# nelpy/ghost

Hardware: NVIDIA B200
Metric: cwt_output_coeffs_per_sec (higher is better)
Workload: dtype f32

## Files before the change

ghost_b200/csrc/fast_path.cu:

```cuda
#include "plan.h"
#include "common.cuh"
#include "multiplier.cuh"
#include <algorithm>
#include <atomic>
#include <cmath>
#include <cstdio>
#include <cstdlib>
#include <map>
#include <type_traits>

namespace gcwt {

constexpr int kMaxFastLevel = 14;
constexpr int kMaxFullScales = 64;
constexpr double kMaxHaloFrac = 0.45;

__constant__ float c_halfband[kHalfbandOdd];
constexpr int kSmallCoef = (2 + 4 + 8) * kInterpT;
__constant__ float c_interp_small[kSmallCoef];
constexpr int kWideCoef = (4 + 8) * kWideT;
__constant__ float c_interp_wide[kWideCoef];

static double bessel_i0(double x) {
    double sum = 1.0, term = 1.0;
// ... 96 lines not shown

static int full_extent(const gcwt_plan* p, const PlanResponses& pr, int s) {
    const double* g = pr.full(s);
    const double e_tot = filter_energy(p, p->scales[s], kFullN);
    double e_in = 0.0;
    int m = 0;
    for (int nmu = 2; nmu <= 8; nmu *= 2) {
        for (; m < nmu * kBins; ++m) e_in += g[m] * g[m];
        if ((1.0 - e_in / e_tot) < p->band_tol * p->band_tol) return nmu;
    }
    return 16;
}

static int band_width_bins(const gcwt_plan* p, const PlanResponses& pr, int s, int level) {
    const double* g = pr.level(s, level);
    const double e_tot = filter_energy(p, p->scales[s], (int64_t)kChunkDec << level);
    const double budget = 0.5 * p->band_tol * p->band_tol * e_tot;
    int lo = 0, hi = kBins - 1;
    double acc = 0.0;
    while (lo < hi && acc + g[lo] * g[lo] < budget) { acc += g[lo] * g[lo]; ++lo; }
    acc = 0.0;
    while (hi > lo && acc + g[hi] * g[hi] < budget) { acc += g[hi] * g[hi]; --hi; }
    return hi - lo + 1;
}

static int choose_level(const gcwt_plan* p, const PlanResponses& pr, int s) {
    const ScaleInfo& sc = p->scales[s];
    if (!(p->flags & GCWT_FLAG_FORCE_GENERIC)) {
        int lo = kMinFastLevel;
        while (lo <= kMaxFastLevel && (double)(sc.L - 1) > kMaxHaloFrac * (double)((int64_t)kChunkDec << lo)) ++lo;
        int hi = std::min(kMaxFastLevel, ilog2_ceil(sc.L) + 1);
        for (int lev = hi; lev >= lo; --lev)
            if (band_fits(p, pr, s, lev)) return lev;
        if ((double)(sc.L - 1) <= kMaxHaloFrac * kFullN) return -1;
    }
    return -2;
}

static void class_geometry(FastClass& fc) {
    const int64_t d = fc.level >= 0 ? (int64_t(1) << fc.level) : 1;
    const int64_t align = std::max<int64_t>(d, 16);
    const int taps = fc.wide ? kWideT : kInterpT;
    const int64_t lead = fc.interp ? (int64_t)(taps / 2 - 1) << fc.log2u : 0;
    const int64_t tail = fc.interp ? (int64_t)(taps / 2 + 1) << fc.log2u : 0;
    fc.offset = ((fc.lmax / 2 + lead + align - 1) / align) * align;
    fc.hop = ((fc.nc_full - (fc.lmax - 1) / 2 - tail - fc.offset) / align) * align;
// ... 208 lines not shown
    p->guard_gain_h = gain;
    p->guard_q_h = q;
    return GCWT_OK;
}

int fast_plan_build(gcwt_plan* p) {
    design_halfband(p->halfband_odd);
    { int rc = upload_constants(p); if (rc) return rc; }
    {
        std::vector<float2> tw(kFullN);
        for (int k = 0; k < kFullN; ++k) {
            const double a = -2.0 * M_PI * (double)k / (double)kFullN;
            tw[k] = make_float2((float)std::cos(a), (float)std::sin(a));
        }
        GCWT_CUDA_OK(cudaMalloc((void**)&p->d_twiddle, sizeof(float2) * kFullN));
        GCWT_CUDA_OK(cudaMemcpy(p->d_twiddle, tw.data(), sizeof(float2) * kFullN, cudaMemcpyHostToDevice));
    }
    PlanResponses pr;
    { int rc = compute_plan_responses(p, pr); if (rc) return rc; }
    std::vector<double> hb((size_t)(kMaxFastLevel + 1) * kBins, 1.0);
    for (int j = 1; j <= kMaxFastLevel; ++j)
        for (int m = 0; m < kBins; ++m)
            hb[(size_t)j * kBins + m] = halfband_gain(p->halfband_odd, 2.0 * M_PI * (double)m / (double)((int64_t)kChunkDec << j));
    std::map<int, std::vector<int>> by_level;
    p->max_level = 0;
    for (int s = 0; s < p->n_scales; ++s) {
        ScaleInfo& sc = p->scales[s];
        sc.level = choose_level(p, pr, s);
        if (sc.level == -2) p->generic_ids.push_back(s);
        else by_level[sc.level].push_back(s);
        p->max_level = std::max(p->max_level, sc.level);
    }
    for (auto& kv : by_level) {
        const int level = kv.first;
        const std::vector<int>& ids = kv.second;
        const int cap = level >= 0 ? kMaxClassScales : kMaxFullScales;
        for (size_t i0 = 0; i0 < ids.size(); i0 += cap) {
            p->classes.emplace_back();
            FastClass& fc = p->classes.back();
            fc.level = level;
            fc.nc_full = level >= 0 ? ((int64_t)kChunkDec << level) : kFullN;
            fc.scale_ids.assign(ids.begin() + i0, ids.begin() + std::min(ids.size(), i0 + cap));
            fc.lmax = 1;
            for (int id : fc.scale_ids) fc.lmax = std::max(fc.lmax, p->scales[id].L);
            const bool may_interp = p->out_kind != GCWT_OUT_COMPLEX && !(p->flags & GCWT_FLAG_NO_INTERP);
            fc.interp = level >= kInterpMinLevel && may_interp;
            fc.log2u = level - 1;
            int wmax = 1;
            if (level >= 0)
                for (int id : fc.scale_ids) wmax = std::max(wmax, band_width_bins(p, pr, id, level));
            if (may_interp && level >= 2 && level <= kWideMaxLevel) {
                if (512.0 / (double)wmax >= kWideMinOs) { fc.interp = true; fc.wide = true; fc.log2u = level; }
            }
            class_geometry(fc);
            if (fc.hop <= 0) { set_error("planner: non-positive hop"); return GCWT_ERR_ARG; }
            if (fc.wide) {
                const int64_t d = int64_t(1) << level, align = std::max<int64_t>(d, 16), nc2 = 2 * fc.nc_full;
                const int64_t lead = (int64_t)(kWideT / 2 - 1) << fc.log2u, tail = (int64_t)(kWideT / 2 + 1) << fc.log2u;
                fc.offset2 = ((fc.lmax / 2 + lead + align - 1) / align) * align;
                fc.hop2 = ((nc2 - (fc.lmax - 1) / 2 - tail - fc.offset2) / align) * align;
                const int ns2 = (int)fc.scale_ids.size();
                std::vector<float2> tab2((size_t)ns2 * 2 * kBins);
                for (int i = 0; i < ns2; ++i) {
                    const ScaleInfo& sc = p->scales[fc.scale_ids[i]];
                    const double* gsrc = pr.wide2(fc.scale_ids[i], level);
                    for (int m = 0; m < 2 * kBins; ++m) {
                        double g = gsrc[m] / (double)(2 * kChunkDec);
                        for (int j = 1; j <= level; ++j)
                            g /= halfband_gain(p->halfband_odd, 2.0 * M_PI * (double)m / (double)((int64_t)(2 * kChunkDec) << j));
                        double re = g, im = 0.0;
                        if ((sc.L & 1) == 0) {
                            const double ph = -M_PI * (double)m / (double)nc2;
                            re = g * std::cos(ph);
                            im = g * std::sin(ph);
                        }
                        tab2[(size_t)i * 2 * kBins + m] = make_float2((float)re, (float)im);
                    }
                }
                GCWT_CUDA_OK(cudaMalloc((void**)&fc.d_table2, sizeof(float2) * tab2.size()));
                GCWT_CUDA_OK(cudaMemcpy(fc.d_table2, tab2.data(), sizeof(float2) * tab2.size(), cudaMemcpyHostToDevice));
            }
            const int nb = level >= 0 ? kBins : kFullN;
            const int ns = (int)fc.scale_ids.size();
            std::vector<float2> tab((size_t)ns * nb);
            for (int i = 0; i < ns; ++i) {
                const ScaleInfo& sc = p->scales[fc.scale_ids[i]];
                const double* gsrc = level >= 0 ? pr.level(fc.scale_ids[i], level) : pr.full(fc.scale_ids[i]);
                for (int m = 0; m < nb; ++m) {
                    double g = gsrc[m];
                    if (level >= 0) {
                        for (int j = 1; j <= level; ++j) g /= hb[(size_t)j * kBins + m];
                        g /= (double)kChunkDec;
                    } else {
                        g /= (double)kFullN;
                    }
                    double re = g, im = 0.0;
                    if ((sc.L & 1) == 0) {
                        const double ph = -M_PI * (double)m / (double)fc.nc_full;
                        re = g * std::cos(ph);
                        im = g * std::sin(ph);
                    }
                    tab[(size_t)i * nb + m] = make_float2((float)re, (float)im);
                }
            }
            GCWT_CUDA_OK(cudaMalloc((void**)&fc.d_table, sizeof(float2) * tab.size()));
            GCWT_CUDA_OK(cudaMemcpy(fc.d_table, tab.data(), sizeof(float2) * tab.size(), cudaMemcpyHostToDevice));
            if (fc.interp) {
                std::vector<float> coef;
                if (fc.wide) {
                    design_interpolator(fc.log2u, coef, kWideT, kWideMinOs);
                } else {
                    const double os = std::min(8.0, std::max(kInterpMinOs, 0.98 * 1024.0 / (double)wmax));
                    design_interpolator(fc.log2u, coef, kInterpT, os);
                }
                GCWT_CUDA_OK(cudaMalloc((void**)&fc.d_coef, sizeof(float) * coef.size()));
                GCWT_CUDA_OK(cudaMemcpy(fc.d_coef, coef.data(), sizeof(float) * coef.size(), cudaMemcpyHostToDevice));
            }
            if (level < 0) {
                for (int id : fc.scale_ids) fc.scale_nmu.push_back(full_extent(p, pr, id));
                GCWT_CUDA_OK(cudaMalloc((void**)&fc.d_scale_nmu, sizeof(int32_t) * ns));
                GCWT_CUDA_OK(cudaMemcpy(fc.d_scale_nmu, fc.scale_nmu.data(), sizeof(int32_t) * ns, cudaMemcpyHostToDevice));
            }
            GCWT_CUDA_OK(cudaMalloc((void**)&fc.d_scale_ids, sizeof(int32_t) * ns));
            GCWT_CUDA_OK(cudaMemcpy(fc.d_scale_ids, fc.scale_ids.data(), sizeof(int32_t) * ns, cudaMemcpyHostToDevice));
        }
    }
    if (p->guard && !p->classes.empty()) {
        if (p->max_level + 2 >= kGuardLevels || (int)p->classes.size() > 64) p->guard = false;
        else { int rc = guard_plan_build(p, pr, hb); if (rc) return rc; }
    } else {
        p->guard = false;
    }
    return GCWT_OK;
}

void fast_plan_free(gcwt_plan* p) {
    if (p->d_guard_gain) cudaFree(p->d_guard_gain);
    if (p->d_guard_q) cudaFree(p->d_guard_q);
    if (p->d_guard_class) cudaFree(p->d_guard_class);
    if (p->d_guard_acc) cudaFree(p->d_guard_acc);
    if (p->d_guard_pow) cudaFree(p->d_guard_pow);
    if (p->d_guard_flags) cudaFree(p->d_guard_flags);
    if (p->h_guard_flags) cudaFreeHost(p->h_guard_flags);
    if (p->ev_guard) cudaEventDestroy(p->ev_guard);
    p->d_guard_gain = p->d_guard_q = nullptr; p->d_guard_class = nullptr; p->d_guard_acc = nullptr;
    p->d_guard_pow = nullptr; p->d_guard_flags = p->h_guard_flags = nullptr; p->ev_guard = nullptr;
    for (auto& fc : p->classes) {
        if (fc.d_table) cudaFree(fc.d_table);
        if (fc.d_table2) cudaFree(fc.d_table2);
        if (fc.d_scale_ids) cudaFree(fc.d_scale_ids);
        if (fc.d_coef) cudaFree(fc.d_coef);
        if (fc.d_scale_nmu) cudaFree(fc.d_scale_nmu);
    }
    p->classes.clear();
}

constexpr int kPyrTile = 1024;

template <typename TIn, bool FIRST>
__global__ void __launch_bounds__(256)
pyramid_kernel(const TIn* __restrict__ in, int64_t in_stride, int64_t in_lo, int64_t in_hi,
               const double* __restrict__ means, float* __restrict__ out, int64_t out_stride,
               int64_t out_lo, int64_t out_len,
               double* __restrict__ acc, int acc_stride, int level, int64_t seg_in, int64_t seg_out) {
    static_assert(kHalfbandT == 19, "tile indexing below assumes kMid == 9");
    constexpr int kMid = (kHalfbandT - 1) / 2;
    constexpr int kEv = kPyrTile + 2 * kMid + 2 + 4;
    constexpr int kOdShift = 12 - kMid;
    __shared__ __align__(16) float ev[kEv];
    __shared__ __align__(16) float ods[kEv + 16];
    const int c = blockIdx.y;
    const int64_t i0 = out_lo + (int64_t)blockIdx.x * kPyrTile;
    const int64_t u0 = 2 * i0 - kHalfbandT;
    const TIn* src = in + (int64_t)c * in_stride - (FIRST ? 0 : in_lo);
    typedef typename std::conditional<std::is_same<TIn, float>::value, float, double>::type TSub;
// ... 63 lines not shown
}

struct FusedParams {
    const void* src;
    int64_t src_stride;
    int64_t src_lo, src_hi;
    const double* means;
    int log2d;
    int p_cols;
    int log2p;
    float inv_nc;
    int64_t offset, hop, n_chunks, n;
    int n_scales;
    const int32_t* scale_ids;
    const float2* table;
    void* out;
    int64_t s_stride, c_stride;
    int iters;
    int units_per_chunk;
    int log2u;
    const float* coef;
    const float2* twf;
    const int32_t* scale_nmu;
    double* acc;
    int acc_stride;
    int class_idx;
    float ech_weight;
    float* pow;
    int pow_stride;
    float pow_weight;
    int guard_every;
    int q_mode;
};

__device__ __forceinline__ float2 tw_pos(const float2* __restrict__ twf, int k) {
    const float2 t = __ldg(twf + (k & (kFullN - 1)));
    return make_float2(t.x, -t.y);
}

__device__ __forceinline__ float sqrt_abs_approx(float v) {
    float r;
    asm("sqrt.approx.ftz.f32 %0, %1;" : "=f"(r) : "f"(fabsf(v)));
    return r;
}

__device__ __forceinline__ float sqrt_approx(float v) {
// ... 53 lines not shown
#pragma unroll
    for (int w = 0; w < 8; ++w) t += scratch[w];
    return t * (1.0f / (float)(NV * 256));
}

template <int NV>
__device__ __forceinline__ void chunk_energy_add(const float* v, float cm, float* scratch, double* dst, float weight) {
    float s = 0.f;
#pragma unroll
    for (int k = 0; k < NV; ++k) { const float d = v[k] - cm; s = fmaf(d, d, s); }
#pragma unroll
    for (int o = 16; o > 0; o >>= 1) s += __shfl_xor_sync(0xffffffffu, s, o);
    __syncthreads();
    if ((threadIdx.x & 31) == 0) scratch[threadIdx.x >> 5] = s;
    __syncthreads();
    if (threadIdx.x == 0) {
        float t = 0.f;
#pragma unroll
        for (int w = 0; w < 8; ++w) t += scratch[w];
        atomicAdd(dst, (double)(t * weight));
    }
}

template <bool PAIRED>
__device__ __forceinline__ void guard_pow_add(const float2* a, unsigned own, float* counter) {
    float pw = 0.f;
#pragma unroll
    for (int k = 0; k < 16; ++k) {
        const float v = a[k].x * a[k].x + a[k].y * a[k].y;
        pw += (own >> k & 1u) ? v : 0.f;
    }
    pw += __shfl_xor_sync(0xffffffffu, pw, 16);
    if (!PAIRED) pw += __shfl_xor_sync(0xffffffffu, pw, 8);
    pw += __shfl_xor_sync(0xffffffffu, pw, 4);
    pw += __shfl_xor_sync(0xffffffffu, pw, 2);
    pw += __shfl_xor_sync(0xffffffffu, pw, 1);
    const unsigned lane = threadIdx.x & 31u;
    if ((lane & (PAIRED ? 23u : 31u)) == 0) atomicAdd(counter, pw);
}

__device__ __forceinline__ float2* smem_fft1024_forward(float2* a, float2* b, const float2* __restrict__ tw) {
    constexpr int M = 256;
    const int j = threadIdx.x;
    float2 w[4][3];
#pragma unroll
    for (int p = 1; p < 5; ++p) {
        const int ns = 1 << (2 * p);
        const int idx = (j & (ns - 1)) * ((kFullN / 4) / ns);
#pragma unroll
        for (int r = 0; r < 3; ++r) w[p - 1][r] = __ldg(tw + (r + 1) * idx);
    }
#pragma unroll
    for (int p = 0; p < 5; ++p) {
        const int ns = 1 << (2 * p);
        const int k = j & (ns - 1);
        float2 v0 = a[j], v1 = a[j + M], v2 = a[j + 2 * M], v3 = a[j + 3 * M];
        if (p > 0) {
            v1 = cmul(v1, w[p - 1][0]);
            v2 = cmul(v2, w[p - 1][1]);
            v3 = cmul(v3, w[p - 1][2]);
        }
// ... 122 lines not shown
        const unsigned mask = valid_mask(rel, lp + 4, own_lo, own_hi);
        for (int s = 0; s < prm.n_scales; ++s) {
            float2 a[16];
            const float2* z = Zs + s * kBins + g;
#pragma unroll
            for (int i = 0; i < 16; ++i) a[i] = cmul(z[16 * i], R[i]);
            dft16<+1>(a);
            float2* e = ex + buf * 4096 + (g * 16) * 16 + r;
            e[0] = a[0];
#pragma unroll
            for (int k = 1; k < 16; ++k) e[k * 16] = cmul(a[k], tw[k]);
            __syncthreads();
            if (pend >= 0 && tid == 0) {
                atomicAdd(pow_c + s_ids[pend], s_pow[pend & 1] * (float)iters * prm.pow_weight);
                s_pow[pend & 1] = 0.f;
            }
            pend = -1;
            const float2* e2 = ex + buf * 4096 + g * 16 + r;
#pragma unroll
            for (int k = 0; k < 16; ++k) a[k] = e2[k * 256];
            dft16<+1>(a);
            store_column<KIND>(out_c + (int64_t)s_ids[s] * prm.s_stride + rel, kstride, mask, a);
            if (GUARD && pow_c != nullptr && it == 0) {
                guard_pow_add<false>(a, mask, s_pow + (s & 1));
                pend = s;
            }
            buf ^= 1;
        }
#pragma unroll
        for (int i = 0; i < 16; ++i) R[i] = cmul(R[i], Estep[g + 16 * i]);
    }
    if (pend >= 0) {
        __syncthreads();
        if (tid == 0) atomicAdd(pow_c + s_ids[pend], s_pow[pend & 1] * (float)iters * prm.pow_weight);
    }
}

constexpr int kPcStride = kCoarse + 16;
constexpr int kPcFloats = 2 * kPcStride;
constexpr size_t kInterpSmem = sizeof(float2) * (4096 + kMaxClassScales * kBins) + sizeof(float) * kPcFloats + sizeof(int) * kMaxClassScales + 16;

template <int KIND, int LU, int T>
__device__ __forceinline__ void interp_rows(const float* __restrict__ pc, float* __restrict__ row,
                                            const float* __restrict__ coef, const float* c0, int lu_rt,
                                            int ia, int ib, int own_hi) {
    const int lu = LU > 0 ? LU : lu_rt;
    const int U = 1 << lu;
// ... 261 lines not shown
            const int iota = (g + 16 * k) * NCOL + col;
            own |= (unsigned)(iota >= ia && iota < ib) << k;
        }
    }
    for (int pair = 0; pair < prm.n_scales; pair += NSC) {
        const int s = min(pair + sidx, prm.n_scales - 1);
        float2 a[16];
        const float2* z = Zs + s * kBins + g;
#pragma unroll
        for (int i = 0; i < 16; ++i) a[i] = cmul(z[16 * i], R[i]);
        dft16<+1>(a);
        float2* e = ex + (g * 16) * 16 + r;
        e[0] = a[0];
#pragma unroll
        for (int k = 1; k < 16; ++k) e[k * 16] = cmul(a[k], tw[k]);
        __syncthreads();
        const float2* e2 = ex + g * 16 + r;
#pragma unroll
        for (int k = 0; k < 16; ++k) a[k] = e2[k * 256];
        dft16<+1>(a);
        float* pc = Pc + sidx * PCS + g * NCOL + col;
#pragma unroll
        for (int k = 0; k < 16; ++k) pc[k * 16 * NCOL] = a[k].x * a[k].x + a[k].y * a[k].y;
        if (sample) guard_pow_add<true>(a, own, s_pow + sidx);
        __syncthreads();
        const int nsc = min(NSC, prm.n_scales - pair);
        if (sample && tid < NSC) {
            if (tid < nsc) atomicAdd(prm.pow + c * prm.pow_stride + s_ids[pair + tid], s_pow[tid] * (float)(1 << lu) * prm.pow_weight);
            s_pow[tid] = 0.f;
        }
        for (int sl = 0; sl < nsc; ++sl) {
            const float* pcs = Pc + sl * PCS;
            float* row = out_c + (int64_t)s_ids[pair + sl] * prm.s_stride;
            if (lu == 2) {
                interp_rows_small<KIND, 2>(pcs, row, ia, ib, own_hi);
            } else if (lu == 1) {
                interp_rows_small<KIND, 1>(pcs, row, ia, ib, own_hi);
            } else {
                switch (lu) {
#ifdef GCWT_L4_SLIDING
                    case 3:  interp_rows<KIND, 3, kInterpT>(pcs, row, prm.coef, c0, lu, ia, ib, own_hi); break;
#else
                    case 3:
                        if (prm.iters == 2 && prm.units_per_chunk == 1) interp_rows_pairs8<KIND>(pcs, row, ia, ib, own_hi, 2);
                        else interp_rows<KIND, 3, kInterpT>(pcs, row, prm.coef, c0, lu, ia, ib, own_hi);
                        break;
#endif
// ... 123 lines not shown
            v[1] = cadd(z0, zr);            v[5] = csub(z0, zr);
            v[3] = cadd(z0, mul_i<+1>(zr)); v[7] = csub(z0, mul_i<+1>(zr));
#pragma unroll
            for (int k = 0; k < 8; ++k)
                A[tid * 17 + sl * 8 + k] = k ? cmul(v[k], tw2k[k]) : v[k];
        }
        __syncthreads();
        float2 a[16];
#pragma unroll
        for (int i = 0; i < 16; ++i) a[i] = A[(g + 16 * i) * 17 + r];
        dft16<+1>(a);
        float2* e = ex + (g * 16) * 16 + r;
        e[0] = a[0];
#pragma unroll
        for (int k = 1; k < 16; ++k) e[k * 16] = cmul(a[k], tw[k]);
        __syncthreads();
        const float2* e2 = ex + g * 16 + r;
#pragma unroll
        for (int k = 0; k < 16; ++k) a[k] = e2[k * 256];
        dft16<+1>(a);
        float* pc = Pc + sidx * kPcStride + g * 8 + col;
#pragma unroll
        for (int k = 0; k < 16; ++k) pc[k * 128] = a[k].x * a[k].x + a[k].y * a[k].y;
        if (sample) guard_pow_add<true>(a, own, s_pow + sidx);
        __syncthreads();
        if (sample && tid < 2) {
            if (pair + tid < prm.n_scales)
                atomicAdd(prm.pow + c * prm.pow_stride + s_ids[pair + tid], s_pow[tid] * (float)(1 << lu) * prm.pow_weight);
            s_pow[tid] = 0.f;
        }
        for (int sl = 0; sl < 2 && pair + sl < prm.n_scales; ++sl) {
            const float* pcs = Pc + sl * kPcStride;
            float* row = out_c + (int64_t)s_ids[pair + sl] * prm.s_stride;
#ifdef GCWT_WIDE_SINGLE
            if (lu == 2) interp_rows_wide<KIND, 2>(pcs, row, ia, ib, own_hi, aligned);
            else interp_rows_wide<KIND, 3>(pcs, row, ia, ib, own_hi, aligned);
#else
            (void)aligned;
            if (lu == 2) interp_rows_wide_pairs<KIND, 2, 2>(pcs, row, ia, ib, own_hi, align);
            else interp_rows_wide_pairs<KIND, 3, 2>(pcs, row, ia, ib, own_hi, align);
#endif
        }
        __syncthreads();
    }
}

constexpr size_t kFullSmem = sizeof(float2) * (2 * 4096 + kTileA) + sizeof(int) * 2 * kMaxFullScales + 16;
// ... 63 lines not shown
            unsigned short* o16 = (unsigned short*)(out_c + (int64_t)s_ids[s] * prm.s_stride) + rel;
#pragma unroll
            for (int k = 0; k < 16; ++k)
                if (mask & (1u << k)) o16[k * 512] = (unsigned short)__float_as_uint(a[k].x * a[k].x + a[k].y * a[k].y);
        }
#elif defined(GCWT_EXP_V2STORE)
        {
            float2* o2 = (float2*)(out_c + (int64_t)s_ids[s] * prm.s_stride) + rel;
#pragma unroll
            for (int k = 0; k < 16; k += 2)
                if (mask & (1u << k)) o2[(k >> 1) * 256] = make_float2(a[k].x * a[k].x + a[k].y * a[k].y, a[k + 1].x * a[k + 1].x + a[k + 1].y * a[k + 1].y);
        }
#elif defined(GCWT_EXP_STSSTORE)
        {
            float* stage = (float*)const_cast<float2*>(Yf);
#pragma unroll
            for (int k = 0; k < 16; ++k) stage[k * 256 + rel] = sqrt_approx(a[k].x * a[k].x + a[k].y * a[k].y);
        }
#elif defined(GCWT_EXP_L2STORE)
        store_column<KIND>((typename out_elem<KIND>::type*)prm.out + (blockIdx.x & 255) * 4096 + rel, 256, mask, a);
#else
        store_column<KIND>(out_c + (int64_t)s_ids[s] * prm.s_stride + rel, 256, mask, a);
#endif
        if (MEASURE) guard_pow_add<false>(a, mask, s_pow + (s & 1));
    }
    if (MEASURE) {
        __syncthreads();
        const int s = prm.n_scales - 1;
        if (tid == 0) atomicAdd(prm.pow + (blockIdx.x / prm.n_chunks) * prm.pow_stride + s_ids[s], s_pow[s & 1] * prm.pow_weight);
    }
}

template <typename TIn, int KIND, bool GUARD>
__global__ void __launch_bounds__(256, 2)
fused_full_kernel(const FusedParams prm) {
    extern __shared__ __align__(16) unsigned char smem_raw[];
    float2* Yf = (float2*)smem_raw;
    float2* ex = Yf + kFullN;
    float2* A = ex + kFullN;
    int* s_ids = (int*)(A + kTileA);
    int* s_nmu = s_ids + kMaxFullScales;
    float* s_pow = (float*)(s_nmu + kMaxFullScales);

    const int tid = threadIdx.x;
    if (tid < 2) s_pow[tid] = 0.f;
    const int r = tid & 15;
    const int g = tid >> 4;
    const int64_t qi = blockIdx.x % prm.n_chunks;
    const int64_t c = blockIdx.x / prm.n_chunks;
    const int64_t q = prm.q_mode == 0 ? qi : (prm.q_mode == 1 ? qi * prm.guard_every : qi + qi / (prm.guard_every - 1) + 1);
    const int64_t t0 = q * prm.hop - prm.offset;

    {
        const TIn* src = (const TIn*)prm.src + c * prm.src_stride;
        const double mu = prm.means[c];
        TIn raw[kFullN / 256];
        unsigned inside = 0;
#pragma unroll
        for (int k = 0; k < kFullN / 256; ++k) {
            const int64_t u = t0 + tid + 256 * k;
            const bool ok = u >= prm.src_lo && u < prm.src_hi;
            raw[k] = ok ? src[u] : (TIn)0;
            inside |= (unsigned)ok << k;
        }
        float val[kFullN / 256];
#pragma unroll
        for (int k = 0; k < kFullN / 256; ++k)
            val[k] = (inside >> k & 1) ? (float)((double)raw[k] - mu) : 0.f;
        const float cm = chunk_mean<kFullN / 256>(val, (float*)ex + 2048);
        if (GUARD)
            chunk_energy_add<kFullN / 256>(val, cm, (float*)ex + 2048, prm.acc + c * prm.acc_stride + kGuardLevels + prm.class_idx,
                                           prm.ech_weight);
#pragma unroll
        for (int k = 0; k < kFullN / 256; ++k) A[tid + 256 * k] = make_float2(val[k] - cm, 0.f);
        __syncthreads();
        smem_fft4096_forward(A, Yf, prm.twf);
    }
    float2 tw[16], tw4k[16];
#pragma unroll
    for (int k = 0; k < 16; ++k) {
        tw[k] = tw_pos(prm.twf, 16 * g * k);
        tw4k[k] = tw_pos(prm.twf, tid * k);
    }
    typedef typename out_elem<KIND>::type OutT;
    const int rel = g * 16 + r;
    const unsigned mask = valid_mask(rel, 8, (int)prm.offset, (int)min(prm.offset + prm.hop, prm.n - t0));
    OutT* const out_c = (OutT*)prm.out + c * prm.c_stride + t0;
    if (tid < prm.n_scales) { s_ids[tid] = prm.scale_ids[tid]; s_nmu[tid] = prm.scale_nmu[tid]; }
    __syncthreads();
    full_scale_loop<KIND, GUARD>(prm, Yf, ex, A, s_ids, s_nmu, s_pow, tw, tw4k, out_c, rel, mask);
}

template <int KIND, int LP, bool GUARD>
static void launch_banded_g(unsigned nblk, cudaStream_t st, const FusedParams& prm) {
    static std::atomic<bool> attr_set[64];
    int dev = 0;
    cudaGetDevice(&dev);
    if (!attr_set[dev & 63]) {
        cudaFuncSetAttribute(fused_banded_kernel<KIND, LP, GUARD>, cudaFuncAttributeMaxDynamicSharedMemorySize, (int)kBandedSmem);
        attr_set[dev & 63] = true;
    }
    fused_banded_kernel<KIND, LP, GUARD><<<nblk, 256, kBandedSmem, st>>>(prm);
}

template <int KIND, int LP>
static void launch_banded_one(unsigned nblk, cudaStream_t st, const FusedParams& prm) {
    if (prm.pow != nullptr) launch_banded_g<KIND, LP, true>(nblk, st, prm);
    else launch_banded_g<KIND, LP, false>(nblk, st, prm);
}

static void launch_banded(int kind, int lp, unsigned nblk, cudaStream_t st, const FusedParams& prm) {
    if (kind == GCWT_OUT_COMPLEX) {
        if (lp == 4) launch_banded_one<GCWT_OUT_COMPLEX, 4>(nblk, st, prm);
// ... 10 lines not shown
template <typename TIn, int KIND, bool GUARD>
static void launch_full_g(unsigned nblk, cudaStream_t st, const FusedParams& prm) {
    static std::atomic<bool> attr_set[64];
    int dev = 0;
    cudaGetDevice(&dev);
    if (!attr_set[dev & 63]) {
        cudaFuncSetAttribute(fused_full_kernel<TIn, KIND, GUARD>, cudaFuncAttributeMaxDynamicSharedMemorySize, (int)kFullSmem);
        attr_set[dev & 63] = true;
    }
    fused_full_kernel<TIn, KIND, GUARD><<<nblk, 256, kFullSmem, st>>>(prm);
}

template <typename TIn, int KIND>
static void launch_full_kind(unsigned nblk, cudaStream_t st, const FusedParams& prm, bool measure) {
    if (measure) launch_full_g<TIn, KIND, true>(nblk, st, prm);
    else launch_full_g<TIn, KIND, false>(nblk, st, prm);
}

template <typename TIn>
static void launch_full(int kind, unsigned nblk, cudaStream_t st, const FusedParams& prm, bool measure) {
    if (kind == GCWT_OUT_COMPLEX) launch_full_kind<TIn, GCWT_OUT_COMPLEX>(nblk, st, prm, measure);
    else if (kind == GCWT_OUT_AMPLITUDE) launch_full_kind<TIn, GCWT_OUT_AMPLITUDE>(nblk, st, prm, measure);
    else launch_full_kind<TIn, GCWT_OUT_POWER>(nblk, st, prm, measure);
}

struct LevelGeom { int64_t lo, hi, len, stride; float* ptr; };

template <typename TIn>
static int fast_run(gcwt_plan* p, const TIn* x, int in_type, int64_t n_channels, int64_t n,
                    int64_t x_stride, int64_t halo_l, int64_t halo_r, const double* d_means,
                    void* out, int64_t s_stride, int64_t c_stride, cudaStream_t st) {
    const bool guard = p->guard;
    const int acc_stride = kGuardLevels + (int)p->classes.size();
    if (guard) {
        if (p->guard_cap < n_channels) {
            if (p->d_guard_acc) cudaFree(p->d_guard_acc);
            if (p->d_guard_pow) cudaFree(p->d_guard_pow);
            if (p->d_guard_flags) cudaFree(p->d_guard_flags);
            if (p->h_guard_flags) cudaFreeHost(p->h_guard_flags);
            p->d_guard_acc = nullptr; p->d_guard_pow = nullptr; p->d_guard_flags = p->h_guard_flags = nullptr; p->guard_cap = 0;
            GCWT_CUDA_OK(cudaMalloc((void**)&p->d_guard_acc, sizeof(double) * acc_stride * n_channels));
            GCWT_CUDA_OK(cudaMalloc((void**)&p->d_guard_pow, sizeof(float) * p->n_scales * n_channels));
            GCWT_CUDA_OK(cudaMalloc((void**)&p->d_guard_flags, (size_t)p->n_scales * n_channels));
            GCWT_CUDA_OK(cudaMallocHost((void**)&p->h_guard_flags, (size_t)p->n_scales * n_channels));
            p->guard_cap = n_channels;
        }
// ... 99 lines not shown
            splits = std::min<int64_t>(splits, 24);
            prm.units_per_chunk = (int)splits;
            const int64_t nblk = chunks * splits;
            if (nblk > 0x7fffffffLL) { set_error("fast path: grid too large"); return GCWT_ERR_UNSUPPORTED; }
            if (p->out_kind == GCWT_OUT_AMPLITUDE) {
                if (guard) fused_interp_kernel<GCWT_OUT_AMPLITUDE, true><<<(unsigned)nblk, 256, kInterpSmem, cs>>>(prm);
                else fused_interp_kernel<GCWT_OUT_AMPLITUDE, false><<<(unsigned)nblk, 256, kInterpSmem, cs>>>(prm);
            } else {
                if (guard) fused_interp_kernel<GCWT_OUT_POWER, true><<<(unsigned)nblk, 256, kInterpSmem, cs>>>(prm);
                else fused_interp_kernel<GCWT_OUT_POWER, false><<<(unsigned)nblk, 256, kInterpSmem, cs>>>(prm);
            }
        } else if (fc.level >= 0) {
            const LevelGeom& g = lv[fc.level];
            prm.src = g.ptr; prm.src_stride = g.stride; prm.src_lo = g.lo; prm.src_hi = g.hi;
            prm.log2d = fc.level;
            prm.p_cols = (int)(fc.nc_full / kBins);
            prm.log2p = ilog2_ceil(prm.p_cols);
            const int blocks = prm.p_cols / 16;
            prm.iters = std::min(blocks, 16);
            prm.units_per_chunk = (blocks + prm.iters - 1) / prm.iters;
            const int64_t nblk = n_channels * prm.n_chunks * prm.units_per_chunk;
            if (nblk > 0x7fffffffLL) { set_error("fast path: grid too large"); return GCWT_ERR_UNSUPPORTED; }
            launch_banded(p->out_kind, prm.log2p, (unsigned)nblk, cs, prm);
        } else {
            prm.src = x; prm.src_stride = x_stride; prm.src_lo = -halo_l; prm.src_hi = n + halo_r;
            prm.log2d = 0; prm.p_cols = 16; prm.log2p = 4; prm.iters = 1; prm.units_per_chunk = 1;
            const int64_t nblk = n_channels * prm.n_chunks;
            if (nblk > 0x7fffffffLL) { set_error("fast path: grid too large"); return GCWT_ERR_UNSUPPORTED; }
            if (!guard) {
                launch_full<TIn>(p->out_kind, (unsigned)nblk, cs, prm, false);
            } else {
                const int64_t n_all = prm.n_chunks, n_meas = (n_all + prm.guard_every - 1) / prm.guard_every;
                if (n_all > n_meas) {
                    prm.q_mode = 2; prm.n_chunks = n_all - n_meas;
                    launch_full<TIn>(p->out_kind, (unsigned)(n_channels * prm.n_chunks), cs, prm, false);
                    count_launch();
                }
                prm.q_mode = prm.guard_every > 1 ? 1 : 0; prm.n_chunks = n_meas;
                launch_full<TIn>(p->out_kind, (unsigned)(n_channels * prm.n_chunks), full_meas_stream ? full_meas_stream : cs, prm, true);
            }
        }
        count_launch();
        prof_end(p, sp, cs);
        return GCWT_OK;
    };

// ... 195 lines not shown
```

ghost_b200/csrc/plan.h:

```cpp
#pragma once
#include <cuda_runtime.h>
#include <stdint.h>
#include <vector>
#include "../../include/ghost_cwt.h"

namespace gcwt {

constexpr int kBins = 256;
constexpr int kChunkDec = 1024;
constexpr int kFullN = 4096;
#ifndef GCWT_MAX_CLASS
#define GCWT_MAX_CLASS 16
#endif
#ifndef GCWT_INTERP_T
#define GCWT_INTERP_T 8
#endif
#ifndef GCWT_WIDE_T
#define GCWT_WIDE_T 12
#endif
#ifndef GCWT_INTERP_CTAS
#define GCWT_INTERP_CTAS 2
#endif
constexpr int kMaxClassScales = GCWT_MAX_CLASS;
constexpr int kMinFastLevel = 2;
constexpr int kInterpT = GCWT_INTERP_T;
constexpr int kInterpMinLevel = 3;
constexpr int kCoarse = 2048;
constexpr int kWideT = GCWT_WIDE_T;
constexpr int kWideMaxLevel = 3;
constexpr double kInterpMinOs = 4.0;
constexpr double kWideMinOs = 2.5;
constexpr int kHalfbandT = 19;
constexpr int kHalfbandOdd = (kHalfbandT + 1) / 2;

struct ScaleInfo {
    int64_t L;
    int32_t k_first;
    int32_t n_terms;
    int32_t term_off;
    int32_t level;
};

struct FastClass {
    int level = 0;
    int64_t nc_full = 0;
    int64_t lmax = 0;
    int64_t offset = 0;
    int64_t hop = 0;
    std::vector<int> scale_ids;
    float2* d_table = nullptr;
    int32_t* d_scale_ids = nullptr;
    std::vector<int> scale_nmu;
    int32_t* d_scale_nmu = nullptr;
    bool interp = false;
    bool wide = false;
    float2* d_table2 = nullptr;
    int64_t offset2 = 0, hop2 = 0;
    int log2u = 0;
    float* d_coef = nullptr;
};

constexpr int kGuardSlots = 18;
constexpr int kGuardLevels = 20;
constexpr double kGuardKRound = 6.0;
constexpr double kGuardKStage = 2.0;

struct Workspace {
    void* ptr = nullptr;
    size_t bytes = 0;
};

constexpr int kMaxBands = 64;
constexpr int kMaxBandEntries = 1024;
struct BandTable {
    int32_t n_bands;
    int32_t rows;
// ... 106 lines not shown
```

Baseline: 770.6 billion.

## Add complex-envelope path for full-resolution scales with narrow bands

For full-length (level -1) scales whose spectral support fits a 1024-bin window, the planner now puts them in a new 'env' class. It stores a shifted 1024-bin filter table per scale plus a window offset, and designs a 4x interpolator. The new fused_env_kernel does one 4096-point forward FFT. For each group of four scales it then runs a 1024-point inverse transform over the bin window and interpolates the complex baseband by 4 with paired FMA before writing amplitude or power. This replaces the 4096-point inverse per scale with a smaller one plus interpolation, trading exactness for a planner-checked energy tolerance and adding a new code path.

```diff
diff --git a/ghost_b200/csrc/fast_path.cu b/ghost_b200/csrc/fast_path.cu
--- a/ghost_b200/csrc/fast_path.cu
+++ b/ghost_b200/csrc/fast_path.cu
@@ -142,6 +142,23 @@
     acc = 0.0;
     while (hi > lo && acc + g[hi] * g[hi] < budget) { acc += g[hi] * g[hi]; --hi; }
     return hi - lo + 1;
+}
+
+static bool envelope_window(const gcwt_plan* p, const PlanResponses& pr, int s, int& k_lo, int& width) {
+    const double* g = pr.full(s);
+    const double e_tot = filter_energy(p, p->scales[s], kFullN);
+    const double budget = 0.5 * p->band_tol * p->band_tol * e_tot;
+    int lo = 0, hi = kFullN - 1;
+    double acc = 0.0;
+    while (lo < hi && acc + g[lo] * g[lo] < budget) { acc += g[lo] * g[lo]; ++lo; }
+    acc = 0.0;
+    while (hi > lo && acc + g[hi] * g[hi] < budget) { acc += g[hi] * g[hi]; --hi; }
+    width = hi - lo + 1;
+    if ((double)width > (double)kEnvBins / kWideMinOs) return false;
+    k_lo = (lo + hi + 1) / 2 - kEnvBins / 2;
+    double e_in = 0.0;
+    for (int m = std::max(k_lo, 0); m < std::min(k_lo + kEnvBins, kFullN / 2); ++m) e_in += g[m] * g[m];
+    return (1.0 - e_in / e_tot) < p->band_tol * p->band_tol;
 }
 
 static int choose_level(const gcwt_plan* p, const PlanResponses& pr, int s) {
@@ -396,28 +413,39 @@
     for (int j = 1; j <= kMaxFastLevel; ++j)
         for (int m = 0; m < kBins; ++m)
             hb[(size_t)j * kBins + m] = halfband_gain(p->halfband_odd, 2.0 * M_PI * (double)m / (double)((int64_t)kChunkDec << j));
+    const bool may_interp = p->out_kind != GCWT_OUT_COMPLEX && !(p->flags & GCWT_FLAG_NO_INTERP);
     std::map<int, std::vector<int>> by_level;
+    std::vector<int> env_ids;
+    std::vector<int> klo(p->n_scales, 0), env_width(p->n_scales, 0);
     p->max_level = 0;
     for (int s = 0; s < p->n_scales; ++s) {
         ScaleInfo& sc = p->scales[s];
         sc.level = choose_level(p, pr, s);
         if (sc.level == -2) p->generic_ids.push_back(s);
+        else if (sc.level == -1 && may_interp && envelope_window(p, pr, s, klo[s], env_width[s])) env_ids.push_back(s);
         else by_level[sc.level].push_back(s);
         p->max_level = std::max(p->max_level, sc.level);
     }
+    struct Group { int level; bool env; std::vector<int> ids; };
+    std::vector<Group> groups;
     for (auto& kv : by_level) {
-        const int level = kv.first;
-        const std::vector<int>& ids = kv.second;
+        groups.push_back({kv.first, false, kv.second});
+        if (kv.first == -1 && !env_ids.empty()) groups.push_back({-1, true, env_ids});
+    }
+    if (!by_level.count(-1) && !env_ids.empty()) groups.insert(groups.begin(), {-1, true, env_ids});
+    for (const Group& grp : groups) {
+        const int level = grp.level;
+        const std::vector<int>& ids = grp.ids;
         const int cap = level >= 0 ? kMaxClassScales : kMaxFullScales;
         for (size_t i0 = 0; i0 < ids.size(); i0 += cap) {
             p->classes.emplace_back();
             FastClass& fc = p->classes.back();
             fc.level = level;
+            fc.env = grp.env;
             fc.nc_full = level >= 0 ? ((int64_t)kChunkDec << level) : kFullN;
             fc.scale_ids.assign(ids.begin() + i0, ids.begin() + std::min(ids.size(), i0 + cap));
             fc.lmax = 1;
             for (int id : fc.scale_ids) fc.lmax = std::max(fc.lmax, p->scales[id].L);
-            const bool may_interp = p->out_kind != GCWT_OUT_COMPLEX && !(p->flags & GCWT_FLAG_NO_INTERP);
             fc.interp = level >= kInterpMinLevel && may_interp;
             fc.log2u = level - 1;
             int wmax = 1;
@@ -426,9 +454,13 @@
             if (may_interp && level >= 2 && level <= kWideMaxLevel) {
                 if (512.0 / (double)wmax >= kWideMinOs) { fc.interp = true; fc.wide = true; fc.log2u = level; }
             }
+            if (fc.env) {
+                fc.interp = true; fc.wide = true; fc.log2u = 2;
+                for (int id : fc.scale_ids) { wmax = std::max(wmax, env_width[id]); fc.scale_klo.push_back(klo[id]); }
+            }
             class_geometry(fc);
             if (fc.hop <= 0) { set_error("planner: non-positive hop"); return GCWT_ERR_ARG; }
-            if (fc.wide) {
+            if (fc.wide && !fc.env) {
                 const int64_t d = int64_t(1) << level, align = std::max<int64_t>(d, 16), nc2 = 2 * fc.nc_full;
                 const int64_t lead = (int64_t)(kWideT / 2 - 1) << fc.log2u, tail = (int64_t)(kWideT / 2 + 1) << fc.log2u;
                 fc.offset2 = ((fc.lmax / 2 + lead + align - 1) / align) * align;
@@ -454,13 +486,14 @@
                 GCWT_CUDA_OK(cudaMalloc((void**)&fc.d_table2, sizeof(float2) * tab2.size()));
                 GCWT_CUDA_OK(cudaMemcpy(fc.d_table2, tab2.data(), sizeof(float2) * tab2.size(), cudaMemcpyHostToDevice));
             }
-            const int nb = level >= 0 ? kBins : kFullN;
+            const int nb = fc.env ? kEnvBins : (level >= 0 ? kBins : kFullN);
             const int ns = (int)fc.scale_ids.size();
             std::vector<float2> tab((size_t)ns * nb);
             for (int i = 0; i < ns; ++i) {
                 const ScaleInfo& sc = p->scales[fc.scale_ids[i]];
                 const double* gsrc = level >= 0 ? pr.level(fc.scale_ids[i], level) : pr.full(fc.scale_ids[i]);
-                for (int m = 0; m < nb; ++m) {
+                for (int j = 0; j < nb; ++j) {
+                    const int m = fc.env ? ((fc.scale_klo[i] + j) & (kFullN - 1)) : j;
                     double g = gsrc[m];
                     if (level >= 0) {
                         for (int j = 1; j <= level; ++j) g /= hb[(size_t)j * kBins + m];
@@ -474,12 +507,20 @@
                         re = g * std::cos(ph);
                         im = g * std::sin(ph);
                     }
-                    tab[(size_t)i * nb + m] = make_float2((float)re, (float)im);
+                    tab[(size_t)i * nb + j] = make_float2((float)re, (float)im);
                 }
             }
             GCWT_CUDA_OK(cudaMalloc((void**)&fc.d_table, sizeof(float2) * tab.size()));
             GCWT_CUDA_OK(cudaMemcpy(fc.d_table, tab.data(), sizeof(float2) * tab.size(), cudaMemcpyHostToDevice));
-            if (fc.interp) {
+            if (fc.env) {
+                std::vector<float> coef;
+                design_interpolator(2, coef, kWideT, std::max(kWideMinOs, (double)kEnvBins / (double)wmax));
+                for (int phi = 1; phi < 4; ++phi)
+                    for (int t = 0; t < kWideT; ++t)
+                        fc.env_coef[phi - 1][t] = make_float2(coef[(size_t)phi * kWideT + t], coef[(size_t)phi * kWideT + t]);
+                GCWT_CUDA_OK(cudaMalloc((void**)&fc.d_scale_klo, sizeof(int32_t) * ns));
+                GCWT_CUDA_OK(cudaMemcpy(fc.d_scale_klo, fc.scale_klo.data(), sizeof(int32_t) * ns, cudaMemcpyHostToDevice));
+            } else if (fc.interp) {
                 std::vector<float> coef;
                 if (fc.wide) {
                     design_interpolator(fc.log2u, coef, kWideT, kWideMinOs);
@@ -490,7 +531,7 @@
                 GCWT_CUDA_OK(cudaMalloc((void**)&fc.d_coef, sizeof(float) * coef.size()));
                 GCWT_CUDA_OK(cudaMemcpy(fc.d_coef, coef.data(), sizeof(float) * coef.size(), cudaMemcpyHostToDevice));
             }
-            if (level < 0) {
+            if (level < 0 && !fc.env) {
                 for (int id : fc.scale_ids) fc.scale_nmu.push_back(full_extent(p, pr, id));
                 GCWT_CUDA_OK(cudaMalloc((void**)&fc.d_scale_nmu, sizeof(int32_t) * ns));
                 GCWT_CUDA_OK(cudaMemcpy(fc.d_scale_nmu, fc.scale_nmu.data(), sizeof(int32_t) * ns, cudaMemcpyHostToDevice));
@@ -525,6 +566,7 @@
         if (fc.d_scale_ids) cudaFree(fc.d_scale_ids);
         if (fc.d_coef) cudaFree(fc.d_coef);
         if (fc.d_scale_nmu) cudaFree(fc.d_scale_nmu);
+        if (fc.d_scale_klo) cudaFree(fc.d_scale_klo);
     }
     p->classes.clear();
 }
@@ -634,6 +676,8 @@
     const float* coef;
     const float2* twf;
     const int32_t* scale_nmu;
+    const int32_t* scale_klo;
+    float2 env_coef[3][kWideT];
     double* acc;
     int acc_stride;
     int class_idx;
@@ -733,8 +777,9 @@
     }
 }
 
-template <bool PAIRED>
+template <int NSC>
 __device__ __forceinline__ void guard_pow_add(const float2* a, unsigned own, float* counter) {
+    static_assert(NSC == 1 || NSC == 2 || NSC == 4, "one, two or four scales per pass");
     float pw = 0.f;
 #pragma unroll
     for (int k = 0; k < 16; ++k) {
@@ -742,12 +787,13 @@
         pw += (own >> k & 1u) ? v : 0.f;
     }
     pw += __shfl_xor_sync(0xffffffffu, pw, 16);
-    if (!PAIRED) pw += __shfl_xor_sync(0xffffffffu, pw, 8);
-    pw += __shfl_xor_sync(0xffffffffu, pw, 4);
+    if (NSC == 1) pw += __shfl_xor_sync(0xffffffffu, pw, 8);
+    if (NSC <= 2) pw += __shfl_xor_sync(0xffffffffu, pw, 4);
     pw += __shfl_xor_sync(0xffffffffu, pw, 2);
     pw += __shfl_xor_sync(0xffffffffu, pw, 1);
     const unsigned lane = threadIdx.x & 31u;
-    if ((lane & (PAIRED ? 23u : 31u)) == 0) atomicAdd(counter, pw);
+    constexpr unsigned kScaleBits = NSC == 1 ? 0u : (NSC == 2 ? 8u : 12u);
+    if ((lane & (31u & ~kScaleBits)) == 0) atomicAdd(counter, pw);
 }
 
 __device__ __forceinline__ float2* smem_fft1024_forward(float2* a, float2* b, const float2* __restrict__ tw) {
@@ -916,7 +962,7 @@
             dft16<+1>(a);
             store_column<KIND>(out_c + (int64_t)s_ids[s] * prm.s_stride + rel, kstride, mask, a);
             if (GUARD && pow_c != nullptr && it == 0) {
-                guard_pow_add<false>(a, mask, s_pow + (s & 1));
+                guard_pow_add<1>(a, mask, s_pow + (s & 1));
                 pend = s;
             }
             buf ^= 1;
@@ -1224,7 +1270,7 @@
         float* pc = Pc + sidx * PCS + g * NCOL + col;
 #pragma unroll
         for (int k = 0; k < 16; ++k) pc[k * 16 * NCOL] = a[k].x * a[k].x + a[k].y * a[k].y;
-        if (sample) guard_pow_add<true>(a, own, s_pow + sidx);
+        if (sample) guard_pow_add<2>(a, own, s_pow + sidx);
         __syncthreads();
         const int nsc = min(NSC, prm.n_scales - pair);
         if (sample && tid < NSC) {
@@ -1394,7 +1440,7 @@
         float* pc = Pc + sidx * kPcStride + g * 8 + col;
 #pragma unroll
         for (int k = 0; k < 16; ++k) pc[k * 128] = a[k].x * a[k].x + a[k].y * a[k].y;
-        if (sample) guard_pow_add<true>(a, own, s_pow + sidx);
+        if (sample) guard_pow_add<2>(a, own, s_pow + sidx);
         __syncthreads();
         if (sample && tid < 2) {
             if (pair + tid < prm.n_scales)
@@ -1504,13 +1550,42 @@
 #else
         store_column<KIND>(out_c + (int64_t)s_ids[s] * prm.s_stride + rel, 256, mask, a);
 #endif
-        if (MEASURE) guard_pow_add<false>(a, mask, s_pow + (s & 1));
+        if (MEASURE) guard_pow_add<1>(a, mask, s_pow + (s & 1));
     }
     if (MEASURE) {
         __syncthreads();
         const int s = prm.n_scales - 1;
         if (tid == 0) atomicAdd(prm.pow + (blockIdx.x / prm.n_chunks) * prm.pow_stride + s_ids[s], s_pow[s & 1] * prm.pow_weight);
     }
+}
+
+template <typename TIn>
+__device__ __forceinline__ void full_front_end(const FusedParams& prm, int64_t c, int64_t t0, bool measure,
+                                               float2* Yf, float2* ex, float2* A) {
+    const int tid = threadIdx.x;
+    const TIn* src = (const TIn*)prm.src + c * prm.src_stride;
+    const double mu = prm.means[c];
+    TIn raw[kFullN / 256];
+    unsigned inside = 0;
+#pragma unroll
+    for (int k = 0; k < kFullN / 256; ++k) {
+        const int64_t u = t0 + tid + 256 * k;
+        const bool ok = u >= prm.src_lo && u < prm.src_hi;
+        raw[k] = ok ? src[u] : (TIn)0;
+        inside |= (unsigned)ok << k;
+    }
+    float val[kFullN / 256];
+#pragma unroll
+    for (int k = 0; k < kFullN / 256; ++k)
+        val[k] = (inside >> k & 1) ? (float)((double)raw[k] - mu) : 0.f;
+    const float cm = chunk_mean<kFullN / 256>(val, (float*)ex + 2048);
+    if (measure)
+        chunk_energy_add<kFullN / 256>(val, cm, (float*)ex + 2048, prm.acc + c * prm.acc_stride + kGuardLevels + prm.class_idx,
+                                       prm.ech_weight);
+#pragma unroll
+    for (int k = 0; k < kFullN / 256; ++k) A[tid + 256 * k] = make_float2(val[k] - cm, 0.f);
+    __syncthreads();
+    smem_fft4096_forward(A, Yf, prm.twf);
 }
 
 template <typename TIn, int KIND, bool GUARD>
@@ -1533,31 +1608,7 @@
     const int64_t q = prm.q_mode == 0 ? qi : (prm.q_mode == 1 ? qi * prm.guard_every : qi + qi / (prm.guard_every - 1) + 1);
     const int64_t t0 = q * prm.hop - prm.offset;
 
-    {
-        const TIn* src = (const TIn*)prm.src + c * prm.src_stride;
-        const double mu = prm.means[c];
-        TIn raw[kFullN / 256];
-        unsigned inside = 0;
-#pragma unroll
-        for (int k = 0; k < kFullN / 256; ++k) {
-            const int64_t u = t0 + tid + 256 * k;
-            const bool ok = u >= prm.src_lo && u < prm.src_hi;
-            raw[k] = ok ? src[u] : (TIn)0;
-            inside |= (unsigned)ok << k;
-        }
-        float val[kFullN / 256];
-#pragma unroll
-        for (int k = 0; k < kFullN / 256; ++k)
-            val[k] = (inside >> k & 1) ? (float)((double)raw[k] - mu) : 0.f;
-        const float cm = chunk_mean<kFullN / 256>(val, (float*)ex + 2048);
-        if (GUARD)
-            chunk_energy_add<kFullN / 256>(val, cm, (float*)ex + 2048, prm.acc + c * prm.acc_stride + kGuardLevels + prm.class_idx,
-                                           prm.ech_weight);
-#pragma unroll
-        for (int k = 0; k < kFullN / 256; ++k) A[tid + 256 * k] = make_float2(val[k] - cm, 0.f);
-        __syncthreads();
-        smem_fft4096_forward(A, Yf, prm.twf);
-    }
+    full_front_end<TIn>(prm, c, t0, GUARD, Yf, ex, A);
     float2 tw[16], tw4k[16];
 #pragma unroll
     for (int k = 0; k < 16; ++k) {
@@ -1571,6 +1622,146 @@
     if (tid < prm.n_scales) { s_ids[tid] = prm.scale_ids[tid]; s_nmu[tid] = prm.scale_nmu[tid]; }
     __syncthreads();
     full_scale_loop<KIND, GUARD>(prm, Yf, ex, A, s_ids, s_nmu, s_pow, tw, tw4k, out_c, rel, mask);
+}
+
+constexpr int kEnvStride = kEnvBins + 8;
+static_assert(4 * kEnvStride <= kTileA, "the V rows of a pass must fit the alias tile");
+
+template <int KIND>
+__device__ __forceinline__ float env_out(float2 v) {
+    const float p = v.x * v.x + v.y * v.y;
+    return KIND == GCWT_OUT_AMPLITUDE ? sqrt_approx(p) : p;
+}
+
+__device__ __forceinline__ float2 ffma2(float2 a, float2 b, float2 c) {
+    float2 d;
+    asm("{\n\t.reg .b64 ra, rb, rc, rd;\n\tmov.b64 ra, {%2, %3};\n\tmov.b64 rb, {%4, %5};\n\tmov.b64 rc, {%6, %7};\n\t"
+        "fma.rn.f32x2 rd, ra, rb, rc;\n\tmov.b64 {%0, %1}, rd;\n\t}"
+        : "=f"(d.x), "=f"(d.y) : "f"(a.x), "f"(a.y), "f"(b.x), "f"(b.y), "f"(c.x), "f"(c.y));
+    return d;
+}
+
+template <int KIND>
+__device__ __forceinline__ void interp_env_pairs(const float2* __restrict__ vr, float* __restrict__ row, int ia, int ib,
+                                                 int own_hi, int align, const float2 (&coef)[3][kWideT]) {
+    static_assert(kWideT == 12, "window indexing below assumes 12 taps");
+    for (int iota = ia + 2 * (int)threadIdx.x; iota < ib; iota += 512) {
+        float2 w[14];
+        const float4* p4 = (const float4*)(vr + iota - 6);
+#pragma unroll
+        for (int j = 0; j < 7; ++j) { const float4 t = p4[j]; w[2 * j] = make_float2(t.x, t.y); w[2 * j + 1] = make_float2(t.z, t.w); }
+        float o[8];
+#pragma unroll
+        for (int h = 0; h < 2; ++h) {
+            o[4 * h] = env_out<KIND>(w[6 + h]);
+#pragma unroll
+            for (int phi = 1; phi < 4; ++phi) {
+                float2 acc = ffma2(coef[phi - 1][0], w[1 + h], make_float2(0.f, 0.f));
+#pragma unroll
+                for (int j = 1; j < kWideT; ++j) acc = ffma2(coef[phi - 1][j], w[1 + h + j], acc);
+                o[4 * h + phi] = env_out<KIND>(acc);
+            }
+        }
+        float* op = row + (int64_t)iota * 4;
+        if (align && (iota + 2) * 4 <= own_hi) {
+            if (align == 2) st_v8(op, o);
+            else { ((float4*)op)[0] = make_float4(o[0], o[1], o[2], o[3]); ((float4*)op)[1] = make_float4(o[4], o[5], o[6], o[7]); }
+        } else {
+#pragma unroll
+            for (int i = 0; i < 8; ++i) if (iota * 4 + i < own_hi) op[i] = o[i];
+        }
+    }
+}
+
+template <typename TIn, int KIND, bool GUARD>
+__global__ void __launch_bounds__(256, 2)
+fused_env_kernel(const FusedParams prm) {
+    extern __shared__ __align__(16) unsigned char smem_raw[];
+    float2* Yf = (float2*)smem_raw;
+    float2* ex = Yf + kFullN;
+    float2* A = ex + kFullN;
+    int* s_ids = (int*)(A + kTileA);
+    int* s_klo = s_ids + kMaxFullScales;
+    float* s_pow = (float*)(s_klo + kMaxFullScales);
+
+    const int tid = threadIdx.x;
+    if (tid < 4) s_pow[tid] = 0.f;
+    const int r = tid & 15;
+    const int g = tid >> 4;
+    const int sidx = r >> 2, kap = r & 3;
+    const int64_t q = blockIdx.x % prm.n_chunks;
+    const int64_t c = blockIdx.x / prm.n_chunks;
+    const int64_t t0 = q * prm.hop - prm.offset;
+    const int own_lo = (int)prm.offset;
+    const int own_hi = (int)min(prm.offset + prm.hop, prm.n - t0);
+    const int ia = own_lo >> 2, ib = (own_hi + 3) >> 2;
+    const bool sample = GUARD && (q % prm.guard_every) == 0;
+
+    full_front_end<TIn>(prm, c, t0, sample, Yf, ex, A);
+    float2 tw[16], tw1k[4];
+#pragma unroll
+    for (int k = 0; k < 16; ++k) tw[k] = tw_pos(prm.twf, 16 * g * k);
+#pragma unroll
+    for (int k = 0; k < 4; ++k) tw1k[k] = tw_pos(prm.twf, 4 * tid * k);
+    if (tid < prm.n_scales) { s_ids[tid] = prm.scale_ids[tid]; s_klo[tid] = prm.scale_klo[tid]; }
+    unsigned own = 0;
+    if (sample) {
+#pragma unroll
+        for (int k = 0; k < 16; ++k) {
+            const int j = 4 * (g + 16 * k) + kap;
+            own |= (unsigned)(j >= ia && j < ib) << k;
+        }
+    }
+    float* const out_c = (float*)prm.out + c * prm.c_stride + t0;
+    const int align = prm.iters;
+    float2* const V = A;
+    __syncthreads();
+    for (int s0 = 0; s0 < prm.n_scales; s0 += 4) {
+#pragma unroll
+        for (int sl = 0; sl < 4; ++sl) {
+            const int s = min(s0 + sl, prm.n_scales - 1);
+            const float2* tab = prm.table + (int64_t)s * kEnvBins + tid;
+            const int klo = s_klo[s] + tid;
+            float2 v[4];
+#pragma unroll
+            for (int mu = 0; mu < 4; ++mu) {
+                const int e = 256 * ((mu + 2) & 3);
+                v[mu] = cmul(Yf[(klo + e) & (kFullN - 1)], __ldg(tab + e));
+            }
+            dft4<+1>(v[0], v[1], v[2], v[3]);
+            A[tid * 17 + 4 * sl] = v[0];
+#pragma unroll
+            for (int k = 1; k < 4; ++k) A[tid * 17 + 4 * sl + k] = cmul(v[k], tw1k[k]);
+        }
+        __syncthreads();
+        float2 a[16];
+#pragma unroll
+        for (int i = 0; i < 16; ++i) a[i] = A[(g + 16 * i) * 17 + r];
+        dft16<+1>(a);
+        float2* e = ex + (g * 16) * 16 + r;
+        e[0] = a[0];
+#pragma unroll
+        for (int k = 1; k < 16; ++k) e[k * 16] = cmul(a[k], tw[k]);
+        __syncthreads();
+        const float2* e2 = ex + g * 16 + r;
+#pragma unroll
+        for (int k = 0; k < 16; ++k) a[k] = e2[k * 256];
+        dft16<+1>(a);
+        float2* vp = V + sidx * kEnvStride + 4 * g + kap;
+#pragma unroll
+        for (int k = 0; k < 16; ++k) vp[64 * k] = a[k];
+        if (sample) guard_pow_add<4>(a, own, s_pow + sidx);
+        __syncthreads();
+        if (sample && tid < 4) {
+            if (s0 + tid < prm.n_scales)
+                atomicAdd(prm.pow + c * prm.pow_stride + s_ids[s0 + tid], s_pow[tid] * 4.f * prm.pow_weight);
+            s_pow[tid] = 0.f;
+        }
+        for (int sl = 0; sl < 4 && s0 + sl < prm.n_scales; ++sl)
+            interp_env_pairs<KIND>(V + sl * kEnvStride, out_c + (int64_t)s_ids[s0 + sl] * prm.s_stride, ia, ib, own_hi, align,
+                                   prm.env_coef);
+        __syncthreads();
+    }
 }
 
 template <int KIND, int LP, bool GUARD>
@@ -1627,6 +1818,29 @@
     if (kind == GCWT_OUT_COMPLEX) launch_full_kind<TIn, GCWT_OUT_COMPLEX>(nblk, st, prm, measure);
     else if (kind == GCWT_OUT_AMPLITUDE) launch_full_kind<TIn, GCWT_OUT_AMPLITUDE>(nblk, st, prm, measure);
     else launch_full_kind<TIn, GCWT_OUT_POWER>(nblk, st, prm, measure);
+}
+
+template <typename TIn, int KIND, bool GUARD>
+static void launch_env_g(unsigned nblk, cudaStream_t st, const FusedParams& prm) {
+    static std::atomic<bool> attr_set[64];
+    int dev = 0;
+    cudaGetDevice(&dev);
+    if (!attr_set[dev & 63]) {
+        cudaFuncSetAttribute(fused_env_kernel<TIn, KIND, GUARD>, cudaFuncAttributeMaxDynamicSharedMemorySize, (int)kFullSmem);
+        attr_set[dev & 63] = true;
+    }
+    fused_env_kernel<TIn, KIND, GUARD><<<nblk, 256, kFullSmem, st>>>(prm);
+}
+
+template <typename TIn>
+static void launch_env(int kind, unsigned nblk, cudaStream_t st, const FusedParams& prm, bool guard) {
+    if (kind == GCWT_OUT_AMPLITUDE) {
+        if (guard) launch_env_g<TIn, GCWT_OUT_AMPLITUDE, true>(nblk, st, prm);
+        else launch_env_g<TIn, GCWT_OUT_AMPLITUDE, false>(nblk, st, prm);
+    } else {
+        if (guard) launch_env_g<TIn, GCWT_OUT_POWER, true>(nblk, st, prm);
+        else launch_env_g<TIn, GCWT_OUT_POWER, false>(nblk, st, prm);
+    }
 }
 
 struct LevelGeom { int64_t lo, hi, len, stride; float* ptr; };
@@ -1772,6 +1986,15 @@
             const int64_t nblk = n_channels * prm.n_chunks * prm.units_per_chunk;
             if (nblk > 0x7fffffffLL) { set_error("fast path: grid too large"); return GCWT_ERR_UNSUPPORTED; }
             launch_banded(p->out_kind, prm.log2p, (unsigned)nblk, cs, prm);
+        } else if (fc.env) {
+            prm.src = x; prm.src_stride = x_stride; prm.src_lo = -halo_l; prm.src_hi = n + halo_r;
+            prm.log2d = 0; prm.units_per_chunk = 1;
+            prm.scale_klo = fc.d_scale_klo;
+            std::copy(&fc.env_coef[0][0], &fc.env_coef[0][0] + 3 * kWideT, &prm.env_coef[0][0]);
+            prm.iters = rows_aligned32 ? 2 : (rows_aligned ? 1 : 0);
+            const int64_t nblk = n_channels * prm.n_chunks;
+            if (nblk > 0x7fffffffLL) { set_error("fast path: grid too large"); return GCWT_ERR_UNSUPPORTED; }
+            launch_env<TIn>(p->out_kind, (unsigned)nblk, cs, prm, guard);
         } else {
             prm.src = x; prm.src_stride = x_stride; prm.src_lo = -halo_l; prm.src_hi = n + halo_r;
             prm.log2d = 0; prm.p_cols = 16; prm.log2p = 4; prm.iters = 1; prm.units_per_chunk = 1;
diff --git a/ghost_b200/csrc/plan.h b/ghost_b200/csrc/plan.h
--- a/ghost_b200/csrc/plan.h
+++ b/ghost_b200/csrc/plan.h
@@ -30,6 +30,7 @@
 constexpr int kWideMaxLevel = 3;
 constexpr double kInterpMinOs = 4.0;
 constexpr double kWideMinOs = 2.5;
+constexpr int kEnvBins = 1024;
 constexpr int kHalfbandT = 19;
 constexpr int kHalfbandOdd = (kHalfbandT + 1) / 2;
 
@@ -52,6 +53,10 @@
     int32_t* d_scale_ids = nullptr;
     std::vector<int> scale_nmu;
     int32_t* d_scale_nmu = nullptr;
+    bool env = false;
+    std::vector<int> scale_klo;
+    int32_t* d_scale_klo = nullptr;
+    float2 env_coef[3][kWideT] = {};
     bool interp = false;
     bool wide = false;
     float2* d_table2 = nullptr;
```

Result: slower. 742.5 billion, median of 6 (-3.6%).
